# oscarknagg/wurm

Hardware: AMD Instinct MI355X
Metric: env_steps_per_s (higher is better)
Workload: dtype i32

## Files before the change

wurm_amd/csrc/options.hip:

```cpp
#include <atomic>
#include <cerrno>
#include <cstdlib>
#include <cstring>

#include "options.hpp"
#include "../../include/wurm_hip.h"

namespace wurm {

constexpr Options DEFAULTS = {1ll << 20, 12288, 6144, -1, -1, -1, 12, 0, 2048, 0, -1, 0, 0, 1, -1, -1, 0, 1024, 256};
Options opt = DEFAULTS;
std::atomic<long long> launch_count{0};

namespace {

struct Entry {
    const char *name;
    long long Options::*field;
};

const Entry table[] = {
    {"WURM_GRID_STEP_MIN_CELLS", &Options::grid_step_min_cells},
    {"WURM_LANE_STEP_MIN_ENVS", &Options::lane_step_min_envs},
    {"WURM_LANE_ROLLOUT_MIN_ENVS", &Options::lane_rollout_min_envs},
    {"WURM_LANE_ROLLOUT_EPW", &Options::lane_rollout_epw},
    {"WURM_RESIDENT_MIN_ENVS", &Options::resident_min_envs},
    {"WURM_RESIDENT_EPW", &Options::resident_epw},
    {"WURM_GRID_WAVES_PER_CU", &Options::grid_waves_per_cu},
    {"WURM_POLICY_GENERIC", &Options::policy_generic},
    {"WURM_MULTI_GROUP_MIN_ENVS", &Options::multi_group_min_envs},
    {"WURM_MULTI_GROUP_VARIANT", &Options::multi_group_variant},
    {"WURM_MULTI_GROUP_STEP_WPB", &Options::multi_group_step_wpb},
    {"WURM_MULTI_GROUP_SHAPE", &Options::multi_group_shape},
    {"WURM_GRID_ROTATE", &Options::grid_rotate},
    {"WURM_MULTI_SHAPE_KERNELS", &Options::multi_shape_kernels},
    {"WURM_GRIDWORLD_LANE_EPW", &Options::gridworld_lane_epw},
    {"WURM_GRID_ROLLOUT_MIN_SIZE", &Options::grid_rollout_min_size},
    {"WURM_POLICY_WIDE", &Options::policy_wide},
    {"WURM_S9_PAIR_MAX_ENVS", &Options::s9_pair_max_envs},
    {"WURM_S9_CROP_HELPER_MIN_STEPS", &Options::s9_crop_helper_min_steps},
};

const Entry *find(const char *name)
{
    if (!name) return nullptr;
    for (const Entry &e : table)
        if (strcmp(e.name, name) == 0) return &e;
    return nullptr;
}

bool parse_whole(const char *v, long long &out)
{
    if (!v || !*v) return false;
    errno = 0;
    char *end = nullptr;
    const long long x = strtoll(v, &end, 10);
    if (errno != 0 || end == v) return false;
    while (*end == ' ' || *end == '\t' || *end == '\n') ++end;
    if (*end != '\0') return false;
    out = x;
    return true;
}

__attribute__((constructor)) void read_environment()
{
    for (const Entry &e : table) {
        long long x;
        if (parse_whole(getenv(e.name), x)) opt.*(e.field) = x;
    }
}

}
}

extern "C" {

int wurm_set_option(const char *name, int64_t value)
{
    const wurm::Entry *e = wurm::find(name);
    if (!e) return WURM_ERR_INVALID_ARG;
    wurm::opt.*(e->field) = (long long)value;
    return WURM_OK;
}

int64_t wurm_get_option(const char *name)
{
    const wurm::Entry *e = wurm::find(name);
    return e ? (int64_t)(wurm::opt.*(e->field)) : INT64_MIN;
}

int64_t wurm_launch_count(void) { return (int64_t)wurm::launch_count.load(std::memory_order_relaxed); }

int wurm_reset_option(const char *name)
{
    const wurm::Entry *e = wurm::find(name);
    if (!e) return WURM_ERR_INVALID_ARG;
    wurm::opt.*(e->field) = wurm::DEFAULTS.*(e->field);
    return WURM_OK;
}

}
```

wurm_amd/csrc/options.hpp:

```cpp
#pragma once
#include <atomic>

namespace wurm {

struct Options {
    long long grid_step_min_cells;
    long long lane_step_min_envs;
    long long lane_rollout_min_envs;
    long long lane_rollout_epw;
    long long resident_min_envs;
    long long resident_epw;
    long long grid_waves_per_cu;
    long long policy_generic;
    long long multi_group_min_envs;
    long long multi_group_variant;
    long long multi_group_step_wpb;
    long long multi_group_shape;
    long long grid_rotate;
    long long multi_shape_kernels;
    long long gridworld_lane_epw;
    long long grid_rollout_min_size;
    long long policy_wide;
    long long s9_pair_max_envs;
    long long s9_crop_helper_min_steps;
};

extern Options opt;

extern std::atomic<long long> launch_count;
#define WURM_LAUNCH(...) do { ::wurm::launch_count.fetch_add(1, std::memory_order_relaxed); hipLaunchKernelGGL(__VA_ARGS__); } while (0)

}
```

wurm_amd/csrc/single_kernels.hpp:

```cpp
#pragma once

#include "single_device.hpp"

namespace wurm {

template <int CPL, bool SNAKE>
__global__ __launch_bounds__(256) void step_kernel(StepArgs p)
{
    const int wave = (int)(threadIdx.x >> 6), wpb = (int)(blockDim.x >> 6);
    const long long env = xcd_block(blockIdx.x, gridDim.x) * wpb + wave;
    if (env >= p.N) return;
    if (p.only_flagged && uniform((int)p.done[env]) != (int)GRID_SKIPPED) return;
    signed char *lds = wurm_lds + wave * p.lds_per_wave;
    const int NCH = SNAKE ? 3 : 2;
    const Geo g = make_geo<CPL>(p.S);
    float *envp = p.envs + env * NCH * g.C;
    Env<CPL> e;
    load_state<CPL, SNAKE>(envp, g, e);
    const long long a_in = uniform64(load_action(p.actions, p.act_dtype, env));
    const bool inj = p.inject_food != nullptr;
    const int inj_cell = inj ? uniform(p.inject_food[env]) : -1;
    StepOut out;
    step_core<CPL, SNAKE, true>(e, g, envp, a_in, out, p.seed, p.call, (u64)(p.env_offset + env), inj, inj_cell, lds);
    if (g.lane == 0) {
        if (SNAKE) {
            store_action(p.actions, p.act_dtype, env, out.action);
            p.selfc[env] = (uint8_t)out.selfc;
        }
        p.reward[env] = out.reward;
        p.done[env] = (uint8_t)out.done;
        p.edgec[env] = (uint8_t)out.edgec;
        if (p.done_copy) p.done_copy[env] = (uint8_t)out.done;
    }
    if (p.obs_mode != WURM_OBS_NONE)
        write_obs<CPL, SNAKE>(e, g, out.headcell, p.obs + env * p.obs_elems, p.obs_mode, p.obs_n, lds);
}

template <int CPL, bool SNAKE>
__global__ __launch_bounds__(256) void fused_step_kernel(StepArgs p)
{
    const int wave = (int)(threadIdx.x >> 6), wpb = (int)(blockDim.x >> 6);
    const long long env = xcd_block(blockIdx.x, gridDim.x) * wpb + wave;
    if (env >= p.N) return;
    if (p.only_flagged && uniform((int)p.done[env]) != (int)GRID_SKIPPED) return;
    fused_step_env<CPL, SNAKE>(p, env, wurm_lds + wave * p.lds_per_wave);
}

template <int CPL, bool SNAKE>
__global__ __launch_bounds__(256) void reset_kernel(StepArgs p)
{
    const int wave = (int)(threadIdx.x >> 6), wpb = (int)(blockDim.x >> 6);
    const long long env = xcd_block(blockIdx.x, gridDim.x) * wpb + wave;
    if (env >= p.N) return;
    signed char *lds = wurm_lds + wave * p.lds_per_wave;
    const int NCH = SNAKE ? 3 : 2;
    const Geo g = make_geo<CPL>(p.S);
    float *envp = p.envs + env * NCH * g.C;
    Env<CPL> e;
    const bool d = uniform((int)p.done_in[env]) != 0;
    if (d) {
        const int *inj = p.inject_reset ? p.inject_reset + env * (SNAKE ? 4 : 1) : nullptr;
        reset_core<CPL, SNAKE>(e, g, p.seed, p.call, (u64)(p.env_offset + env), inj, p.start_y, p.start_x);
        store_state<CPL, SNAKE>(envp, g, e);
    } else {
        if (p.obs_mode == WURM_OBS_NONE) return;
        load_state<CPL, SNAKE>(envp, g, e);
    }
    if (p.obs_mode != WURM_OBS_NONE)
        write_obs<CPL, SNAKE>(e, g, find_head<CPL>(e), p.obs + env * p.obs_elems, p.obs_mode, p.obs_n, lds);
}

template <int CPL, bool SNAKE>
__global__ __launch_bounds__(256) void observe_kernel(StepArgs p)
{
    const int wave = (int)(threadIdx.x >> 6), wpb = (int)(blockDim.x >> 6);
    const long long env = xcd_block(blockIdx.x, gridDim.x) * wpb + wave;
    if (env >= p.N) return;
    signed char *lds = wurm_lds + wave * p.lds_per_wave;
    const int NCH = SNAKE ? 3 : 2;
    const Geo g = make_geo<CPL>(p.S);
    Env<CPL> e;
    load_state<CPL, SNAKE>(p.envs + env * NCH * g.C, g, e);
    write_obs<CPL, SNAKE>(e, g, find_head<CPL>(e), p.obs + env * p.obs_elems, p.obs_mode, p.obs_n, lds);
}

template <int CPL, bool SNAKE, int OBSK = -1, bool INJ = true>
__global__ __launch_bounds__(256) void rollout_kernel(StepArgs p)
{
    const int wave = uniform((int)(threadIdx.x >> 6)), wpb = (int)(blockDim.x >> 6);
    const long long env = xcd_block(blockIdx.x, gridDim.x) * wpb + wave;
    if (env >= p.N) return;
    if (p.only_flagged && uniform((int)p.done[env]) != (int)GRID_SKIPPED) return;
    signed char *lds = wurm_lds + wave * p.lds_per_wave;
    const Geo g = make_geo<CPL>(p.S);
    float *envp = p.envs + env * (SNAKE ? 3 : 2) * g.C;
    Env<CPL> e;
    load_state<CPL, SNAKE>(envp, g, e);
    rollout_generic<CPL, SNAKE, OBSK, INJ>(p, env, envp, g, e, lds);
}

template <int CPL, bool SNAKE, bool ROLL>
__global__ __launch_bounds__(256) void flagged_kernel(StepArgs p)
{
    const int wave = uniform((int)(threadIdx.x >> 6)), wpb = (int)(blockDim.x >> 6), lane = (int)(threadIdx.x & 63u);
    const long long base = ((long long)blockIdx.x * wpb + wave) * 64;
    if (base >= p.N) return;
    const bool flag = base + lane < p.N && p.done[base + lane] == GRID_SKIPPED;
    signed char *lds = wurm_lds + wave * p.lds_per_wave;
    for (u64 m = ballot(flag); m != 0; m &= m - 1) {
        const long long env = base + first_bit(m);
        if constexpr (ROLL) {
            const Geo g = make_geo<CPL>(p.S);
            float *envp = p.envs + env * (SNAKE ? 3 : 2) * g.C;
            Env<CPL> e;
            load_state<CPL, SNAKE>(envp, g, e);
            rollout_generic<CPL, SNAKE, -1, true>(p, env, envp, g, e, lds);
        } else {
            fused_step_env<CPL, SNAKE>(p, env, lds);
        }
        wave_lds_sync();
    }
}


template <int OBSK, bool COMPACT>
__global__ __launch_bounds__(256) void rollout_lean_kernel(StepArgs p)
{
    constexpr int CPL = 2;
    static_assert(OBSK == WURM_OBS_PARTIAL || OBSK == WURM_OBS_NONE, "lean rollout: partial_n or no observation");
    const int wave = uniform((int)(threadIdx.x >> 6)), wpb = (int)(blockDim.x >> 6);
    const long long env = xcd_block(blockIdx.x, gridDim.x) * wpb + wave;
    if (env >= p.N) return;
    const Geo g = make_geo<CPL>(p.S);
    const int S = g.S, Sm2 = S - 2, lane = g.lane;
    float *envp = p.envs + env * 3 * g.C;
    Env<CPL> e;
    load_state<CPL, true>(envp, g, e);

    Fast f = {-1, 0, 0, 0, 0, -1};
    bool lean = fast_init<CPL>(e, g, f);
    if (lean) {
        const bool head_in = f.hc >= 0 && (unsigned)(f.hy - 1) < (unsigned)Sm2 && (unsigned)(f.hx - 1) < (unsigned)Sm2;
        int under_food = 0;
        if (f.food >= 0) under_food = lane_value(f.food >= 64 ? e.body[1] : e.body[0], f.food & 63);
        lean = head_in && under_food == 0;
    }
    if (!uniform((int)lean)) {
        rollout_generic<CPL, true, OBSK, false>(p, env, envp, g, e, wurm_lds + wave * p.lds_per_wave);
        return;
    }

    const u64 env_id = (u64)(p.env_offset + env);
    const u64 int0 = ballot((g.interior & 1) != 0), int1 = ballot((g.interior & 2) != 0);
    const float rcpSm2 = 1.0f / (float)Sm2;
    int hy1 = uniform(f.hy) - 1, hx1 = uniform(f.hx) - 1, hc = uniform(f.hc), L = uniform(f.L), o16 = uniform(f.o) << 4;
    int food = uniform(f.food);
    int foodc = food - (COMPACT ? S + 1 : 0);
    int G = L;
    int ex0 = e.body[0], ex1 = e.body[1];
    const u64 ring0 = lane_mask((g.valid & 1) != 0) & ~int0, ring1 = lane_mask((g.valid & 2) != 0) & ~int1;
    u64 X0 = ring0 | ((unsigned)food < 64u ? 1ull << food : 0), X1 = ring1 | (food >= 64 ? 1ull << (food - 64) : 0);

    const int n = OBSK == WURM_OBS_PARTIAL ? p.obs_n : 0, W = 2 * n + 1, W2 = W * W;
    const int w = min(lane, W2 - 1), wy = div_size(w, 1.0f / (float)W), wx = w - wy * W;
    const int dy0 = wy - n, dx0 = wx - n;
    const bool centre = w == n * W + n;
    const int cell_d = dy0 * S + dx0 - (COMPACT ? S + 1 : 0);
    const float green = centre ? 1.0f : 127.0f / 255.0f;
    const u32 off_r = (u32)w * 4u, off_g = (u32)(W2 + w) * 4u, off_b = (u32)(2 * W2 + w) * 4u;
    const long long obs_stride = p.N * p.obs_elems;
    float *obs_t = p.obs + env * p.obs_elems;

    for (long long t0 = 0; t0 < p.T; t0 += 64) {
        const int nt = (int)min((long long)64, p.T - t0);
        const long long my_t = t0 + lane;
        long long my_a = lane < nt ? load_action(p.actions, p.act_dtype, my_t * p.N + env) : 0;
        asm volatile("" : "+v"(my_a));
        int my_mov01, my_mov23;
        {
            const bool in_range = my_a >= 0 && my_a < 4;
            const int a_small = in_range ? (int)my_a : 7, a_mod = (int)(my_a % 4);
            int ent[4];
#pragma unroll
            for (int o = 0; o < 4; ++o) {
                const int a_out = o == a_small ? (o ^ 2) : a_mod;
                const int ai = a_out & 3, dy = -tap_y(ai), dx = -tap_x(ai);
                ent[o] = (a_out & 7) | ((ai ^ 2) << 4) | ((dy & 3) << 6) | ((dx & 3) << 8) | (((dy * S + dx) & 63) << 10);
            }
            my_mov01 = ent[0] | (ent[1] << 16);
            my_mov23 = ent[2] | (ent[3] << 16);
        }
        const u64 my_call = p.call + 2ull * (u64)my_t;
        const LeanReset my_reset = lean_reset_draw(p.seed, my_call + 1ull, env_id, S, rcpSm2);
        const int my_food = (int)rng_words(p.seed, my_call, env_id, RNG_FOOD, 0).w[0];
        int my_rec = 0, my_ate = 0, my_fl = 0;
        {
            const int T = G - L;
            ex0 = max(ex0 - T, 0);
            ex1 = max(ex1 - T, 0);
            G = L;
        }

        for (int j = 0; j < nt; ++j) {
            const u64 mov = (u64)(u32)lane_value(my_mov01, j) | ((u64)(u32)lane_value(my_mov23, j) << 32);
            const int ent = (int)(u32)(mov >> o16);
            o16 = ent & 48;
            hy1 += (ent << 24) >> 30;
            hx1 += (ent << 22) >> 30;
            hc += (ent << 16) >> 26;
            G += 1;
            asm("s_cmp_eq_u32 %1, %2\n\ts_addc_u32 %0, %0, 0" : "+s"(L) : "s"(hc), "s"(food) : "scc");
            const int T = G - L;
            const u64 p0 = lane_mask(ex0 > T), p1 = lane_mask(ex1 > T);
            ex0 = lane == hc ? G : ex0;
            ex1 = lane + 64 == hc ? G : ex1;
            const u64 special = hc >= 64 ? (p1 | X1) : (p0 | X0);
            bool finished = false, selfc = false, edgec = false;
            if (__builtin_expect(((special >> (hc & 63)) & 1) != 0, 0)) {
                if (hc == food) {
                    my_ate = lane == j ? 1 : my_ate;
                    const u64 head0 = (unsigned)hc < 64u ? 1ull << hc : 0, head1 = hc >= 64 ? 1ull << (hc - 64) : 0;
                    food = lean_food_cell(p0 | head0, p1 | head1, int0, int1, (u32)lane_value(my_food, j), lane);
                    foodc = food - (COMPACT ? S + 1 : 0);
                    X0 = ring0 | ((unsigned)food < 64u ? 1ull << food : 0);
                    X1 = ring1 | (food >= 64 ? 1ull << (food - 64) : 0);
                }
                selfc = (((hc >= 64 ? p1 : p0) >> (hc & 63)) & 1) != 0;
                edgec = max((unsigned)hy1, (unsigned)hx1) >= (unsigned)Sm2;
                finished = selfc | edgec;
            }

            if (OBSK == WURM_OBS_PARTIAL) {
                const unsigned off_grid = max((unsigned)(hy1 + dy0), (unsigned)(hx1 + dx0));
                const int cell = (COMPACT && centre) ? 63 : hc + cell_d;
                unsigned occ;
                if (COMPACT) {
                    const u64 M = (p0 >> (S + 1)) | (p1 << (63 - S)) | (1ull << 63);
                    u64 sh;
                    asm("v_lshrrev_b64 %0, %1, %2" : "=v"(sh) : "v"(cell), "s"(M));
                    occ = (u32)sh & 1u;
                } else {
                    occ = ((u32)((cell < 64 ? p0 : p1) >> (cell & 63)) & 1u) | (centre ? 1u : 0u);
                }
                const float vr = (off_grid | (occ << 30)) < (unsigned)Sm2 ? 1.0f : 0.0f;
                const float vb = cell == foodc ? 0.0f : vr;
                const float vg = (off_grid | ((occ ^ 1u) << 30)) < (unsigned)Sm2 ? green : vb;
                asm volatile("global_store_dword %0, %1, %2" : : "v"(off_r), "v"(vr), "s"(obs_t) : "memory");
                asm volatile("global_store_dword %0, %1, %2" : : "v"(off_g), "v"(vg), "s"(obs_t) : "memory");
                asm volatile("global_store_dword %0, %1, %2" : : "v"(off_b), "v"(vb), "s"(obs_t) : "memory");
                obs_t += obs_stride;
            }
            my_rec = set_lane(my_rec, ent, j);

            if (__builtin_expect(finished, 0)) {
                my_fl = lane == j ? (selfc ? 1 : 0) | (edgec ? 2 : 0) : my_fl;
                const int ra = lane_value(my_reset.a, j), rb = lane_value(my_reset.b, j);
                hy1 = (ra & 15) - 1; hx1 = ((ra >> 4) & 15) - 1; o16 = ((ra >> 8) & 3) << 4; food = ra >> 10;
                foodc = food - (COMPACT ? S + 1 : 0);
                X0 = ring0 | ((unsigned)food < 64u ? 1ull << food : 0);
                X1 = ring1 | (food >= 64 ? 1ull << (food - 64) : 0);
                hc = rb & 127;
                const int sc = (rb >> 7) & 127, tc = rb >> 14;
                const int c1 = lane + 64;
                ex0 = lane == tc ? T + 1 : 0; ex0 = lane == sc ? T + 2 : ex0; ex0 = lane == hc ? T + 3 : ex0;
                ex1 = c1 == tc ? T + 1 : 0;   ex1 = c1 == sc ? T + 2 : ex1;   ex1 = c1 == hc ? T + 3 : ex1;
                L = 3;
                G = T + 3;
            }
        }
        if (lane < nt) {
            const long long i = my_t * p.N + env;
            store_action(p.actions, p.act_dtype, i, (long long)((my_rec << 29) >> 29));
            p.reward[i] = my_ate ? 1.0f : 0.0f;
            p.done[i] = (uint8_t)(my_fl != 0);
            p.selfc[i] = (uint8_t)(my_fl & 1);
            p.edgec[i] = (uint8_t)(my_fl >> 1);
        }
    }
    const int T = G - L;
    e.body[0] = max(ex0 - T, 0);
    e.body[1] = max(ex1 - T, 0);
    f.hc = hc; f.hy = hy1 + 1; f.hx = hx1 + 1; f.L = L; f.o = o16 >> 4; f.food = food;
    fast_sync_bits<CPL>(e, g, f);
    store_state<CPL, true>(envp, g, e);
}


template <int OBSK, bool INJ = false, bool PAIR = false, bool CROPH = false>
__global__ __launch_bounds__(256) void rollout_s9_kernel(StepArgs p)
{
    constexpr int CPL = 2, S = 9;
    static_assert(OBSK == WURM_OBS_PARTIAL || OBSK == WURM_OBS_NONE, "9x9 rollout: partial_n or no observation");
    static_assert(!CROPH || (PAIR && OBSK == WURM_OBS_PARTIAL), "9x9 rollout: the helper renders the crops of the pair form");
    const int wave = uniform((int)(threadIdx.x >> 6)), wpb = (int)(blockDim.x >> 6);
    const long long env = PAIR ? xcd_block(blockIdx.x, gridDim.x) : xcd_block(blockIdx.x, gridDim.x) * wpb + wave;
    if (env >= p.N) return;
    const Geo g = make_geo<CPL>(S);
    const int lane = g.lane;
    const u64 env_id = (u64)(p.env_offset + env);
    WURM_TL_DECL;
    WURM_TL(0);
    WURM_TL(6);

    const auto chunk_draw = [&](const long long t0, const int nt) __attribute__((always_inline)) {
        S9Chunk ch;
        const long long my_t = t0 + lane;
        long long my_a = lane < nt ? load_action(p.actions, p.act_dtype, my_t * p.N + env) : 0;
        asm volatile("" : "+v"(my_a));
        if constexpr (!PAIR) WURM_TL_LAP(1);
        {
            const auto entry = [](int a_out) {
                const int ai = a_out & 3;
                return ((ai ^ 2) << 4) | (((-tap_y(ai) * 8 - tap_x(ai)) & 63) << 6) | ((a_out & 7) << 12);
            };
            const bool in_range = my_a >= 0 && my_a < 4;
            const int a_small = in_range ? (int)my_a : 7, a_mod = (int)(my_a % 4);
            int me[4];
#pragma unroll
            for (int o = 0; o < 4; ++o)
                me[o] = entry(o == a_small ? (o ^ 2) : a_mod);
            ch.mov01 = me[0] | (me[1] << 16);
            ch.mov23 = me[2] | (me[3] << 16);
        }
        const u64 my_call = p.call + 2ull * (u64)my_t;
        if constexpr (INJ) {
            int sy = 4, sx = 4, d = 0, fc = -1, fe = -1;
            if (lane < nt) {
                const int *ir = p.inject_reset + (my_t * p.N + env) * 4;
                sy = ir[0]; sx = ir[1]; d = ir[2]; fc = ir[3];
                fe = p.inject_food[my_t * p.N + env];
            }
            asm volatile("" : "+v"(sy), "+v"(sx), "+v"(d), "+v"(fc), "+v"(fe));
            d &= 3;
            const int sc = sy * 8 + sx, dc = tap_y(d) * 8 + tap_x(d);
            const int fcy = div_size(max(fc, 0), g.rcpS), fey = div_size(max(fe, 0), g.rcpS);
            const int fcode = (fc >= 0 && fc < S * S) ? fcy * 8 + (fc - fcy * S) : -1;
            ch.reset.a = d | (fcode << 2);
            ch.reset.b = (sc + dc) | (sc << 7) | ((sc - dc) << 14);
            ch.food = (fe >= 0 && fe < S * S) ? fey * 8 + (fe - fey * S) : -1;
        } else {
            ch.reset = s9_reset_draw(p.seed, my_call + 1ull, env_id);
            ch.food = (int)rng_words(p.seed, my_call, env_id, RNG_FOOD, 0).w[0];
        }
        return ch;
    };
    const auto flush = [&](const long long t0, const int nt, const int act, const int ate, const int fl) __attribute__((always_inline)) {
        if (lane < nt) {
            const long long i = (t0 + lane) * p.N + env;
            store_action(p.actions, p.act_dtype, i, (long long)act);
            p.reward[i] = ate ? 1.0f : 0.0f;
            p.done[i] = (uint8_t)(fl != 0);
            p.selfc[i] = (uint8_t)(fl & 1);
            p.edgec[i] = (uint8_t)(fl >> 1);
        }
    };

    int *const pair_lds = (int *)(wurm_lds + p.lds_per_wave);
    constexpr int PAIR_CHUNK = 5 * 64, PAIR_REC = 2 * PAIR_CHUNK, PAIR_RECSZ = CROPH ? 4 * 64 : 64, PAIR_LEAN = PAIR_REC + 2 * PAIR_RECSZ;
    const long long n_chunks = (p.T + 63) >> 6;
    if constexpr (PAIR) {
        if (wave != 0) {
            const auto draw_into = [&](const long long k) __attribute__((always_inline)) {
                const long long t0 = k << 6;
                const S9Chunk ch = chunk_draw(t0, (int)min((long long)64, p.T - t0));
                int *cb = pair_lds + (int)(k & 1) * PAIR_CHUNK + lane;
                cb[0] = ch.mov01; cb[64] = ch.mov23; cb[128] = ch.reset.a; cb[192] = ch.reset.b; cb[256] = ch.food;
            };
            const auto flush_from = [&](const long long k) __attribute__((always_inline)) {
                const long long t0 = k << 6;
                const int rec = pair_lds[PAIR_REC + (int)(k & 1) * PAIR_RECSZ + lane];
                flush(t0, (int)min((long long)64, p.T - t0), (rec << 29) >> 29, (rec >> 3) & 1, rec >> 4);
            };
            int spp = 1, sub = 0;
            S9Window win = {};
            if constexpr (CROPH) {
#ifndef WURM_S9_CROP_SPP1
                spp = (2 * p.obs_n + 1) * (2 * p.obs_n + 1) <= 32 ? 2 : 1;
#endif
                sub = spp == 2 ? lane >> 5 : 0;
                win = s9_window(spp == 2 ? lane & 31 : lane, p.obs_n);
            }
            const auto render = [&](const long long k) __attribute__((always_inline)) {
                const int W2 = (2 * p.obs_n + 1) * (2 * p.obs_n + 1);
                const long long t0 = k << 6, obs_stride = p.N * p.obs_elems;
                const int nt = (int)min((long long)64, p.T - t0);
                const int *rb = pair_lds + PAIR_REC + (int)(k & 1) * PAIR_RECSZ;
                const int centre = win.code_d == 0 ? 1 : 0, code_d1 = win.code_d + 1;
                float *obs_t = p.obs + (t0 * p.N + env) * p.obs_elems;
                const auto pass = [&](const int j, const int my_sub) __attribute__((always_inline)) {
                    const int sj = j + my_sub;
                    const int w1 = rb[64 + sj];
                    const u64 body = (u64)(u32)rb[128 + sj] | ((u64)(u32)rb[192 + sj] << 32);
                    const int c = w1 & 127;
                    unsigned inside = (u32)(win.live_tab >> (w1 & 63)) & 1u;
                    const bool edge = ((w1 >> 26) & 1) != 0;
                    if (lane_mask(edge) != 0) {
                        const int ai = (w1 >> 22) & 3, pc = c - ((w1 << 10) >> 26);
                        const int hy = (pc >> 3) - tap_y(ai), hx = (pc & 7) - tap_x(ai);
                        const unsigned e_inside = max((unsigned)(hy + win.dy0 - 1), (unsigned)(hx + win.dx0 - 1)) < 7u ? 1u : 0u;
                        inside = edge ? e_inside : inside;
                    }
                    const unsigned taken = ((u32)(body >> ((w1 + win.code_d) & 63)) & 1u) | (u32)centre;
                    const unsigned both = inside & taken;
                    const int code1 = c + code_d1, food1 = (w1 >> 7) & 127;
                    const float vr = inside > taken ? 1.0f : 0.0f;
                    const float vb = code1 != food1 ? vr : 0.0f;
                    const float vg = both != 0 ? win.green : vb;
                    const u32 o = (u32)((long long)my_sub * obs_stride * 4) + (u32)win.w * 4u;
                    float *const obs_s = (float *)uniform64((long long)obs_t);
                    asm volatile("global_store_dword %0, %1, %6\n\tglobal_store_dword %2, %3, %6\n\tglobal_store_dword %4, %5, %6"
                                 : : "v"(o), "v"(vr), "v"(o + (u32)W2 * 4u), "v"(vg), "v"(o + (u32)W2 * 8u), "v"(vb), "s"(obs_s) : "memory");
                };
                int j = 0;
                for (; j + spp <= nt; j += spp) {
                    pass(j, sub);
                    obs_t += spp * obs_stride;
                }
                if (j < nt) pass(j, 0);
            };
            if (n_chunks > 0) draw_into(0);
            pair_barrier();
            if (uniform(pair_lds[PAIR_LEAN]) == 0) return;
            for (long long k = 0; k < n_chunks; ++k) {
                if (k + 1 < n_chunks) draw_into(k + 1);
                if (k > 0) flush_from(k - 1);
                if constexpr (CROPH) {
                    WURM_TL_LAP(1);
                    if (k > 0) render(k - 1);
                    WURM_TL_LAP(2);
                }
                pair_barrier();
                if constexpr (CROPH) WURM_TL_LAP(3);
            }
            if (n_chunks > 0) flush_from(n_chunks - 1);
            if constexpr (CROPH) {
                WURM_TL_LAP(1);
                if (n_chunks > 0) render(n_chunks - 1);
                WURM_TL_LAP(4);
                if (p.T > 1) WURM_TL_STORE(p.obs + (p.N + env) * p.obs_elems, lane);
            }
            return;
        }
    }

    float *envp = p.envs + env * 3 * (S * S);
    Env<CPL> e;
    load_state<CPL, true>(envp, g, e);

    Fast f = {-1, 0, 0, 0, 0, -1};
    bool lean = fast_init<CPL>(e, g, f);
    if (lean) {
        const bool head_in = f.hc >= 0 && (unsigned)(f.hy - 1) < 7u && (unsigned)(f.hx - 1) < 7u;
        const int fy = f.food >= 0 ? div_size(f.food, g.rcpS) : 1, fx = f.food >= 0 ? f.food - fy * S : 1;
        const bool food_in = (unsigned)(fy - 1) < 7u && (unsigned)(fx - 1) < 7u;
        int under_food = 0;
        if (f.food >= 0) under_food = lane_value(f.food >= 64 ? e.body[1] : e.body[0], f.food & 63);
        const bool ring_body = lane_mask((e.body[0] > 0 && !(g.interior & 1)) || (e.body[1] > 0 && !(g.interior & 2))) != 0;
        lean = head_in && food_in && under_food == 0 && !ring_body;
    }
    if constexpr (PAIR) {
        if (lane == 0) pair_lds[PAIR_LEAN] = lean ? 1 : 0;
        pair_barrier();
    }
    if (!uniform((int)lean)) {
        rollout_generic<CPL, true, OBSK, INJ, true>(p, env, envp, g, e, wurm_lds + wave * p.lds_per_wave);
        return;
    }

    const int ly = lane >> 3, lx = lane & 7;
    const bool lane_in = ly >= 1 && lx >= 1;
    const int my_cell = ly * S + lx;
    const u64 RING = ~lane_mask(lane_in);
    int ex = lane_in ? __float2int_rn(envp[2 * S * S + my_cell]) : 0;
    int c = uniform(f.hy) * 8 + uniform(f.hx), ent = uniform(f.o) << 4;
    int foodc = -1;
    if (f.food >= 0) {
        const int fy = uniform(div_size(f.food, g.rcpS));
        foodc = fy * 8 + (uniform(f.food) - fy * S);
    }
    u64 XF = RING | (foodc >= 0 ? 1ull << foodc : 0);
    int G = uniform(f.L), T1 = 1;

    const int n = OBSK == WURM_OBS_PARTIAL ? p.obs_n : 0, W = 2 * n + 1, W2 = W * W;
    const int w = min(lane, W2 - 1), wy = div_size(w, 1.0f / (float)W), wx = w - wy * W;
    const int dy0 = wy - n, dx0 = wx - n;
    const int code_d = dy0 * 8 + dx0;
    const float green = (w == n * W + n) ? 1.0f : 127.0f / 255.0f;
    u64 live_tab = 0;
#pragma unroll
    for (int y = 1; y <= 7; ++y) {
        u32 cols = 0;
#pragma unroll
        for (int x = 1; x <= 7; ++x)
            if ((unsigned)(x + dx0 - 1) < 7u) cols |= 1u << x;
        if ((unsigned)(y + dy0 - 1) < 7u) live_tab |= (u64)cols << (8 * y);
    }
    const u32 off_r = (u32)w * 4u, off_g = (u32)(W2 + w) * 4u, off_b = (u32)(2 * W2 + w) * 4u;
    const long long obs_stride = p.N * p.obs_elems;
    float *obs_t = p.obs + env * p.obs_elems;

    WURM_TL_LAP(5);
    for (long long t0 = 0; t0 < p.T; t0 += 64) {
        const int nt = (int)min((long long)64, p.T - t0);
        int my_mov01, my_mov23, my_food;
        S9Reset my_reset;
        if constexpr (PAIR) {
            const int *cb = pair_lds + (int)((t0 >> 6) & 1) * PAIR_CHUNK + lane;
            my_mov01 = cb[0]; my_mov23 = cb[64]; my_reset.a = cb[128]; my_reset.b = cb[192]; my_food = cb[256];
            asm volatile("" : "+v"(my_mov01), "+v"(my_mov23), "+v"(my_reset.a), "+v"(my_reset.b), "+v"(my_food));
            WURM_TL_LAP(1);
        } else {
            const S9Chunk ch = chunk_draw(t0, nt);
            my_mov01 = ch.mov01; my_mov23 = ch.mov23; my_reset = ch.reset; my_food = ch.food;
#ifdef WURM_TIMELINE
            asm volatile("" : "+v"(my_mov01), "+v"(my_mov23), "+v"(my_reset.a), "+v"(my_reset.b), "+v"(my_food));
#endif
            WURM_TL_LAP(2);
        }
        int my_rec = 0, my_ate = 0, my_fl = 0;
        S9CropRec crop_rec = {0, 0, 0, 0, 0};
        {
            const int T = T1 - 1;
            ex = max(ex - T, 0);
            G -= T;
            T1 = 1;
        }

        const auto step = [&](const int j) __attribute__((always_inline)) {
            const u64 body_moved = lane_mask(ex > T1);
            const u64 mov = (u64)(u32)lane_value(my_mov01, j) | ((u64)(u32)lane_value(my_mov23, j) << 32);
            ent = (int)(u32)(mov >> (ent & 63));
            if constexpr (!CROPH) my_rec = set_lane(my_rec, ent, j);
            asm("s_add_i32 %0, %0, %1" : "+s"(c) : "s"((ent << 20) >> 26) : "scc");
            G += 1;
            asm("s_cmp_lg_u32 %1, %2\n\ts_addc_u32 %0, %0, 0" : "+s"(T1) : "s"(c), "s"(foodc) : "scc");
            if constexpr (CROPH) set_lane(crop_rec, ent, c, foodc, body_moved, j);
            u64 body = body_moved;
            const u64 head = 1ull << (c & 63);
            ex = keep_in_lane(ex, G, head);
            u64 occ = body | head;

            unsigned inside = 0;
            int code = c + code_d;
            u64 mask = occ;
            if (OBSK == WURM_OBS_PARTIAL && !CROPH) {
                u64 lv;
                asm("v_lshrrev_b64 %0, %1, %2" : "=v"(lv) : "s"(c), "v"(live_tab));
                inside = (u32)lv & 1u;
            }

            int shown_food = foodc;
            if (__builtin_expect((((body | XF) >> (c & 63)) & 1) != 0, 0)) {
                const u64 lane_j = 1ull << (j & 63);
                if (c == foodc) {
                    my_ate = keep_in_lane(my_ate, 1, lane_j);
                    occ = lane_mask(ex > T1 - 1);
                    body = occ & ~head;
                    mask = occ;
                    if constexpr (INJ) {
                        foodc = lane_value(my_food, j);
                    } else {
                        const u64 fr = ~(occ | RING);
                        const int n_free = popc64(fr);
                        foodc = -1;
                        if (n_free > 0) {
                            const int K = (int)mulhi_range((u32)lane_value(my_food, j), (u32)n_free);
                            foodc = first_bit(lane_mask((int)((fr >> lane) & 1) & (int)(rank_below(fr) == K)));
                        }
                    }
                    XF = RING | (foodc >= 0 ? 1ull << foodc : 0);
                    if constexpr (CROPH) {
                        crop_rec.food = set_lane(crop_rec.food, foodc, j);
                        crop_rec.body_lo = set_lane(crop_rec.body_lo, (int)(u32)body, j);
                        crop_rec.body_hi = set_lane(crop_rec.body_hi, (int)(u32)(body >> 32), j);
                    }
                }
                shown_food = foodc;
                const int event = ((RING >> (c & 63)) & 1) ? 2 : ((body >> (c & 63)) & 1) ? 1 : 0;
                if (OBSK == WURM_OBS_PARTIAL && !CROPH && event == 2) {
                    const int ai = (ent >> 12) & 3, pc = c - ((ent << 20) >> 26);
                    const int hy = (pc >> 3) - tap_y(ai), hx = (pc & 7) - tap_x(ai);
                    inside = max((unsigned)(hy + dy0 - 1), (unsigned)(hx + dx0 - 1)) < 7u ? 1u : 0u;
                    code = (hy + dy0) * 8 + hx + dx0;
                    mask = body;
                }
                if (event != 0) {
                    my_fl = keep_in_lane(my_fl, event, lane_j);
                    const int ra = lane_value(my_reset.a, j), rb = lane_value(my_reset.b, j);
                    ent = (ra & 3) << 4;
                    foodc = ra >> 2;
                    XF = INJ ? (RING | (foodc >= 0 ? 1ull << foodc : 0)) : (RING | (1ull << foodc));
                    c = rb & 127;
                    const int sc = (rb >> 7) & 127, tc = rb >> 14;
                    ex = lane == tc ? T1 : 0; ex = lane == sc ? T1 + 1 : ex; ex = lane == c ? T1 + 2 : ex;
                    G = T1 + 2;
                }
            }

            if (OBSK == WURM_OBS_PARTIAL && !CROPH) {
                u64 sh;
                asm("v_lshrrev_b64 %0, %1, %2" : "=v"(sh) : "v"(code), "s"(mask));
                const unsigned taken = (u32)sh & 1u;
                const unsigned both = inside & taken;
                float vr, vb, vg;
                u64 m_free, m_not_food, m_taken;
                asm("v_cmp_gt_u32_e64 %3, %6, %7\n\t"
                    "v_cmp_ne_u32_e64 %4, %8, %9\n\t"
                    "v_cmp_ne_u32_e64 %5, 0, %10\n\t"
                    "v_cndmask_b32_e64 %0, 0, 1.0, %3\n\t"
                    "v_cndmask_b32_e64 %1, 0, %0, %4\n\t"
                    "v_cndmask_b32_e64 %2, %1, %11, %5"
                    : "=&v"(vr), "=&v"(vb), "=&v"(vg), "=&s"(m_free), "=&s"(m_not_food), "=&s"(m_taken)
                    : "v"(inside), "v"(taken), "s"(shown_food), "v"(code), "v"(both), "v"(green));
                asm volatile("global_store_dword %0, %1, %6\n\tglobal_store_dword %2, %3, %6\n\tglobal_store_dword %4, %5, %6"
                             : : "v"(off_r), "v"(vr), "v"(off_g), "v"(vg), "v"(off_b), "v"(vb), "s"(obs_t) : "memory");
                obs_t += obs_stride;
            }
        };
        constexpr int U = 4;
        const int nu = nt & -U;
        int j = 0;
        for (; j != nu; j += U) {
#pragma unroll
            for (int u = 0; u < U; ++u) step(j + u);
        }
        for (; j < nt; ++j) step(j);
        WURM_TL_LAP(3);
        if constexpr (PAIR) {
            if constexpr (CROPH) {
                int *rb = pair_lds + PAIR_REC + (int)((t0 >> 6) & 1) * PAIR_RECSZ + lane;
                my_rec = crop_rec.ent;
                rb[64] = (crop_rec.c & 127) | (((crop_rec.food + 1) & 127) << 7) | (((my_rec >> 4) & 0x7FF) << 14) | ((my_fl & 3) << 25);
                rb[128] = crop_rec.body_lo;
                rb[192] = crop_rec.body_hi;
                rb[0] = ((my_rec >> 12) & 7) | (my_ate << 3) | (my_fl << 4);
            } else {
                pair_lds[PAIR_REC + (int)((t0 >> 6) & 1) * 64 + lane] = ((my_rec >> 12) & 7) | (my_ate << 3) | (my_fl << 4);
            }
            pair_barrier();
        } else {
            flush(t0, nt, (my_rec << 17) >> 29, my_ate, my_fl);
        }
        WURM_TL_LAP(4);
    }
    if (OBSK == WURM_OBS_PARTIAL && (!CROPH || p.T > 64)) WURM_TL_STORE(p.obs + env * p.obs_elems, lane);
    if (lane_in) {
        envp[my_cell] = lane == foodc ? 1.0f : 0.0f;
        envp[S * S + my_cell] = lane == c ? 1.0f : 0.0f;
        envp[2 * S * S + my_cell] = (float)max(ex - (T1 - 1), 0);
    }
}

template <int CPL>
__global__ __launch_bounds__(256) void check_kernel(const float *__restrict__ envs, uint32_t *__restrict__ err,
                                                    long long N, int S)
{
    const int wave = (int)(threadIdx.x >> 6), wpb = (int)(blockDim.x >> 6);
    const long long env = xcd_block(blockIdx.x, gridDim.x) * wpb + wave;
    if (env >= N) return;
    const Geo g = make_geo<CPL>(S);
    const float *envp = envs + env * 3 * g.C;
    int bad_food = 0;
    float hs = 0.0f, bs = 0.0f, bm = -INFINITY, hb = 0.0f, hf = 0.0f, fs = 0.0f;
#pragma unroll
    for (int k = 0; k < CPL; ++k) {
        int c = g.lane + 64 * k;
        if ((g.valid >> k) & 1) {
            float f = envp[c], h = envp[g.C + c], b = envp[2 * g.C + c];
            bad_food |= !(f == 0.0f || f == 1.0f);
            hs += h; bs += b; hb += h * b; hf += h * f; fs += f;
            bm = fmaxf(bm, b);
        }
    }
    bad_food = ballot(bad_food != 0) != 0;
#pragma unroll
    for (int sh = 32; sh >= 1; sh >>= 1) {
        hs += __shfl_xor(hs, sh); bs += __shfl_xor(bs, sh); hb += __shfl_xor(hb, sh); hf += __shfl_xor(hf, sh);
        fs += __shfl_xor(fs, sh); bm = fmaxf(bm, __shfl_xor(bm, sh));
    }
    uint32_t m = 0;
    if (bad_food) m |= WURM_CHK_FOOD_VALUE;
    if (hs != 1.0f) m |= WURM_CHK_ONE_HEAD;
    if (!(bs > 0.0f)) m |= WURM_CHK_HAS_SNAKE;
    if (bm != hb) m |= WURM_CHK_HEAD_AT_END;
    if ((__fsqrt_rn(8.0f * bs + 1.0f) - 1.0f) / 2.0f != bm) m |= WURM_CHK_BODY_RANGE;
    if (!(bs >= 6.0f)) m |= WURM_CHK_MIN_LENGTH;
    if (hf != 0.0f) m |= WURM_CHK_HEAD_ON_FOOD;
    if (fs != 1.0f) m |= WURM_CHK_ONE_FOOD;
    if (g.lane == 0) err[env] = m;
}

template <int CPL>
__global__ __launch_bounds__(256) void orientations_kernel(const float *__restrict__ envs, long long *__restrict__ out,
                                                           long long N, int S, int lds_per_wave)
{
    const int wave = (int)(threadIdx.x >> 6), wpb = (int)(blockDim.x >> 6);
    const long long env = xcd_block(blockIdx.x, gridDim.x) * wpb + wave;
    if (env >= N) return;
    signed char *lds = wurm_lds + wave * lds_per_wave;
    const Geo g = make_geo<CPL>(S);
    Env<CPL> e;
    load_state<CPL, true>(envs + env * 3 * g.C, g, e);
    int lm = 0;
#pragma unroll
    for (int k = 0; k < CPL; ++k) lm = max(lm, e.body[k]);
    const int L = uniform(wave_max_i32(lm));
    const int o = orientation_of<CPL>(e, g, L, lds);
    if (g.lane == 0) out[env] = o;
}

}
```

wurm_amd/csrc/single_launch.hpp:

```cpp
#pragma once

#include "single_kernels.hpp"
#include "lane_step.hpp"

namespace wurm {

enum Kind { K_STEP, K_RESET, K_OBSERVE, K_ROLLOUT, K_FUSED };

enum Route { R_GENERIC, R_GRID_STEP, R_LANE_STEP, R_GRID_ROLLOUT, R_LANE_ROLLOUT, R_LANE_WIDE, R_S9_INJ, R_S9, R_LEAN, R_GENERIC_PARTIAL, R_GENERIC_NONE, R_LANE_RESIDENT, R_LANE_WIDE_RESIDENT, R_GRIDWORLD_LANE, R_GRIDWORLD_LANE_STEP };
extern thread_local Route last_route;
extern thread_local int last_waves_per_env;
extern thread_local int last_crop_wave;

static const char *route_name(Route r)
{
    switch (r) {
    case R_GRID_STEP: return "grid_step";
    case R_LANE_STEP: return "lane_step";
    case R_GRID_ROLLOUT: return "grid_rollout";
    case R_LANE_ROLLOUT: return "lane_rollout";
    case R_LANE_WIDE: return "lane_wide";
    case R_S9_INJ: return "rollout_s9_injected";
    case R_S9: return "rollout_s9";
    case R_LEAN: return "rollout_lean";
    case R_GENERIC_PARTIAL: return "rollout_generic_partial";
    case R_GENERIC_NONE: return "rollout_generic_none";
    case R_LANE_RESIDENT: return "lane_resident";
    case R_LANE_WIDE_RESIDENT: return "lane_wide_resident";
    case R_GRIDWORLD_LANE: return "gridworld_lane";
    case R_GRIDWORLD_LANE_STEP: return "gridworld_lane_step";
    default: return "generic";
    }
}

static Route route_of(Kind kind, bool snake, int cpl, const StepArgs &p)
{
    const bool stepish = kind == K_STEP || kind == K_FUSED;
    if (snake && cpl >= 4 && stepish && grid_step_eligible(p) &&
        (p.N * (long long)p.S * p.S >= opt.grid_step_min_cells || p.resident != nullptr)) return R_GRID_STEP;
    if (snake && cpl == 2 && stepish && p.N >= opt.lane_step_min_envs && lane_step_eligible(p)) return R_LANE_STEP;
    if (kind == K_ROLLOUT && !snake && gridworld_lane_eligible(p)) return R_GRIDWORLD_LANE;
    if (stepish && !snake && gridworld_lane_step_eligible(p)) return R_GRIDWORLD_LANE_STEP;
    if (kind != K_ROLLOUT || !snake) return R_GENERIC;
    if (cpl >= 4) return grid_rollout_eligible(p) ? R_GRID_ROLLOUT : R_GENERIC;
    if (p.N >= opt.lane_rollout_min_envs && lane_rollout_eligible(p)) return R_LANE_ROLLOUT;
    if (p.N >= opt.lane_rollout_min_envs && lane_wide_eligible(p)) return R_LANE_WIDE;
    const bool rng_mode = p.inject_food == nullptr && p.inject_reset == nullptr;
    const bool injected = p.inject_food != nullptr && p.inject_reset != nullptr;
    const bool small_crop_or_none = (p.obs_mode == WURM_OBS_PARTIAL && p.obs_n <= 3) || p.obs_mode == WURM_OBS_NONE;
    if (injected && p.S == 9 && small_crop_or_none) return R_S9_INJ;
    if (rng_mode && p.S == 9 && small_crop_or_none) return R_S9;
    if (rng_mode && p.S > 9 && small_crop_or_none) return R_LEAN;
    if (rng_mode && p.obs_mode == WURM_OBS_PARTIAL && p.obs_n <= 6) return R_GENERIC_PARTIAL;
    if (rng_mode && p.obs_mode == WURM_OBS_NONE) return R_GENERIC_NONE;
    return R_GENERIC;
}

template <int CPL, bool SNAKE>
static hipError_t launch_one(Kind kind, const StepArgs &p, dim3 grid, dim3 block, size_t lds, hipStream_t st)
{
    (void)hipGetLastError();
    const Route route = route_of(kind, SNAKE, CPL, p);
    last_route = route;
    last_waves_per_env = 1;
    last_crop_wave = 0;
    const unsigned wpb_f = block.x / 64u;
    const dim3 fgrid((unsigned)((p.N + 64ll * wpb_f - 1) / (64ll * wpb_f)));
    switch (route) {
    case R_GRID_STEP:
        if constexpr (SNAKE && CPL >= 4) {
            hipError_t err = launch_grid_step(p, st);
            if (err != hipSuccess) return err;
            WURM_LAUNCH((flagged_kernel<CPL, SNAKE, false>), fgrid, block, lds, st, p);
        }
        break;
    case R_LANE_STEP:
        if constexpr (SNAKE && CPL == 2) return launch_lane_step(p, st);
        break;
    case R_GRID_ROLLOUT:
        if constexpr (SNAKE && CPL >= 4) {
            hipError_t err = launch_grid_rollout(p, st);
            if (err != hipSuccess) return err;
            WURM_LAUNCH((flagged_kernel<CPL, SNAKE, true>), fgrid, block, lds, st, p);
        }
        break;
    case R_LANE_ROLLOUT:
        if constexpr (SNAKE && CPL == 2) return launch_lane_rollout(p, st);
        break;
    case R_LANE_WIDE:
        if constexpr (SNAKE && CPL == 2) return launch_lane_wide(p, st);
        break;
    case R_GRIDWORLD_LANE:
        if constexpr (!SNAKE) {
            hipError_t err = launch_gridworld_lane_rollout(p, st);
            if (err != hipSuccess) return err;
            if (!(p.resident != nullptr && p.resident_valid))
                WURM_LAUNCH((flagged_kernel<CPL, SNAKE, true>), fgrid, block, lds, st, p);
        }
        break;
    case R_GRIDWORLD_LANE_STEP:
        if constexpr (!SNAKE) {
            hipError_t err = launch_gridworld_lane_step(p, st);
            if (err != hipSuccess) return err;
            if (!(p.resident != nullptr && p.resident_valid))
                WURM_LAUNCH((flagged_kernel<CPL, SNAKE, false>), fgrid, block, lds, st, p);
        }
        break;
    case R_S9_INJ:
    case R_S9:
        if constexpr (SNAKE && CPL == 2) {
            const bool inj = route == R_S9_INJ, none = p.obs_mode == WURM_OBS_NONE;
            if (p.N <= opt.s9_pair_max_envs) {
                const dim3 pgrid((unsigned)p.N), pblock(128);
                const size_t plds = (size_t)p.lds_per_wave + (2 * 5 * 64 + 2 * 64 + 4) * sizeof(int);
                last_waves_per_env = 2;
                if (!none && opt.s9_crop_helper_min_steps >= 0 && p.T >= opt.s9_crop_helper_min_steps &&
                    p.N * p.obs_elems * 4 < (1ll << 31)) {
                    const size_t clds = (size_t)p.lds_per_wave + (2 * 5 * 64 + 2 * 4 * 64 + 4) * sizeof(int);
                    last_crop_wave = 1;
                    if (inj) WURM_LAUNCH((rollout_s9_kernel<WURM_OBS_PARTIAL, true, true, true>), pgrid, pblock, clds, st, p);
                    else WURM_LAUNCH((rollout_s9_kernel<WURM_OBS_PARTIAL, false, true, true>), pgrid, pblock, clds, st, p);
                } else
                if (inj && none) WURM_LAUNCH((rollout_s9_kernel<WURM_OBS_NONE, true, true>), pgrid, pblock, plds, st, p);
                else if (inj) WURM_LAUNCH((rollout_s9_kernel<WURM_OBS_PARTIAL, true, true>), pgrid, pblock, plds, st, p);
                else if (none) WURM_LAUNCH((rollout_s9_kernel<WURM_OBS_NONE, false, true>), pgrid, pblock, plds, st, p);
                else WURM_LAUNCH((rollout_s9_kernel<WURM_OBS_PARTIAL, false, true>), pgrid, pblock, plds, st, p);
            } else if (inj) {
                if (none) WURM_LAUNCH((rollout_s9_kernel<WURM_OBS_NONE, true>), grid, block, lds, st, p);
                else WURM_LAUNCH((rollout_s9_kernel<WURM_OBS_PARTIAL, true>), grid, block, lds, st, p);
            } else {
                if (none) WURM_LAUNCH((rollout_s9_kernel<WURM_OBS_NONE>), grid, block, lds, st, p);
                else WURM_LAUNCH((rollout_s9_kernel<WURM_OBS_PARTIAL>), grid, block, lds, st, p);
            }
        }
        break;
    case R_LEAN:
        if constexpr (SNAKE && CPL == 2) {
            if (p.obs_mode == WURM_OBS_NONE) WURM_LAUNCH((rollout_lean_kernel<WURM_OBS_NONE, false>), grid, block, lds, st, p);
            else WURM_LAUNCH((rollout_lean_kernel<WURM_OBS_PARTIAL, false>), grid, block, lds, st, p);
        }
        break;
    case R_GENERIC_PARTIAL:
        if constexpr (SNAKE && CPL == 2) WURM_LAUNCH((rollout_kernel<CPL, SNAKE, WURM_OBS_PARTIAL, false>), grid, block, lds, st, p);
        break;
    case R_GENERIC_NONE:
        if constexpr (SNAKE && CPL == 2) WURM_LAUNCH((rollout_kernel<CPL, SNAKE, WURM_OBS_NONE, false>), grid, block, lds, st, p);
        break;
    case R_LANE_RESIDENT:
    case R_LANE_WIDE_RESIDENT:
    case R_GENERIC:
        switch (kind) {
        case K_STEP: WURM_LAUNCH((step_kernel<CPL, SNAKE>), grid, block, lds, st, p); break;
        case K_RESET: WURM_LAUNCH((reset_kernel<CPL, SNAKE>), grid, block, lds, st, p); break;
        case K_OBSERVE: WURM_LAUNCH((observe_kernel<CPL, SNAKE>), grid, block, lds, st, p); break;
        case K_FUSED: WURM_LAUNCH((fused_step_kernel<CPL, SNAKE>), grid, block, lds, st, p); break;
        case K_ROLLOUT: WURM_LAUNCH((rollout_kernel<CPL, SNAKE>), grid, block, lds, st, p); break;
        }
        break;
    }
    return hipGetLastError();
}

template <bool SNAKE>
int launch(Kind kind, StepArgs p, void *stream)
{
    if (p.N == 0) return WURM_OK;
    const int cpl = pick_cpl(p.S);
    if (cpl < 0) return WURM_ERR_UNSUPPORTED;
    const int wpb = p.N <= 4096 ? 1 : 4;
    p.lds_per_wave = ((p.S * p.S + 15) / 16) * 16;
    dim3 block(64 * wpb), grid((unsigned)((p.N + wpb - 1) / wpb));
    size_t lds = (size_t)p.lds_per_wave * wpb;
    hipStream_t st = (hipStream_t)stream;
    hipError_t err;
    switch (cpl) {
    case 2: err = launch_one<2, SNAKE>(kind, p, grid, block, lds, st); break;
    case 4: err = launch_one<4, SNAKE>(kind, p, grid, block, lds, st); break;
    case 8: err = launch_one<8, SNAKE>(kind, p, grid, block, lds, st); break;
    case 16: err = launch_one<16, SNAKE>(kind, p, grid, block, lds, st); break;
    case 24: err = launch_one<24, SNAKE>(kind, p, grid, block, lds, st); break;
    case 32: err = launch_one<32, SNAKE>(kind, p, grid, block, lds, st); break;
    case 48: err = launch_one<48, SNAKE>(kind, p, grid, block, lds, st); break;
    default: err = launch_one<64, SNAKE>(kind, p, grid, block, lds, st); break;
    }
    return err == hipSuccess ? WURM_OK : WURM_ERR_HIP;
}

}
```

Baseline: 4.418 billion.

## Add third render-only wave to 9x9 pair rollout for small env counts

After: 4.874 billion (median of 6 runs). 1.1x the previous value.

```diff
diff --git a/wurm_amd/csrc/options.hip b/wurm_amd/csrc/options.hip
--- a/wurm_amd/csrc/options.hip
+++ b/wurm_amd/csrc/options.hip
@@ -8,7 +8,7 @@
 
 namespace wurm {
 
-constexpr Options DEFAULTS = {1ll << 20, 12288, 6144, -1, -1, -1, 12, 0, 2048, 0, -1, 0, 0, 1, -1, -1, 0, 1024, 256};
+constexpr Options DEFAULTS = {1ll << 20, 12288, 6144, -1, -1, -1, 12, 0, 2048, 0, -1, 0, 0, 1, -1, -1, 0, 1024, 256, 512, 512};
 Options opt = DEFAULTS;
 std::atomic<long long> launch_count{0};
 
@@ -39,6 +39,8 @@
     {"WURM_POLICY_WIDE", &Options::policy_wide},
     {"WURM_S9_PAIR_MAX_ENVS", &Options::s9_pair_max_envs},
     {"WURM_S9_CROP_HELPER_MIN_STEPS", &Options::s9_crop_helper_min_steps},
+    {"WURM_S9_TRIO_MAX_ENVS", &Options::s9_trio_max_envs},
+    {"WURM_S9_TRIO_MIN_STEPS", &Options::s9_trio_min_steps},
 };
 
 const Entry *find(const char *name)
diff --git a/wurm_amd/csrc/options.hpp b/wurm_amd/csrc/options.hpp
--- a/wurm_amd/csrc/options.hpp
+++ b/wurm_amd/csrc/options.hpp
@@ -23,6 +23,8 @@
     long long policy_wide;
     long long s9_pair_max_envs;
     long long s9_crop_helper_min_steps;
+    long long s9_trio_max_envs;
+    long long s9_trio_min_steps;
 };
 
 extern Options opt;
diff --git a/wurm_amd/csrc/single_kernels.hpp b/wurm_amd/csrc/single_kernels.hpp
--- a/wurm_amd/csrc/single_kernels.hpp
+++ b/wurm_amd/csrc/single_kernels.hpp
@@ -286,12 +286,14 @@
 }
 
 
-template <int OBSK, bool INJ = false, bool PAIR = false, bool CROPH = false>
+template <int OBSK, bool INJ = false, bool PAIR = false, bool CROPH = false, int RW = 1>
 __global__ __launch_bounds__(256) void rollout_s9_kernel(StepArgs p)
 {
     constexpr int CPL = 2, S = 9;
+    constexpr int S9_TRIO_SHARE = 24, S9_TRIO_LAST_SHARE = 32;
     static_assert(OBSK == WURM_OBS_PARTIAL || OBSK == WURM_OBS_NONE, "9x9 rollout: partial_n or no observation");
     static_assert(!CROPH || (PAIR && OBSK == WURM_OBS_PARTIAL), "9x9 rollout: the helper renders the crops of the pair form");
+    static_assert(RW == 1 || (RW == 2 && CROPH), "9x9 rollout: a second render wave beside a helper that renders");
     const int wave = uniform((int)(threadIdx.x >> 6)), wpb = (int)(blockDim.x >> 6);
     const long long env = PAIR ? xcd_block(blockIdx.x, gridDim.x) : xcd_block(blockIdx.x, gridDim.x) * wpb + wave;
     if (env >= p.N) return;
@@ -360,6 +362,7 @@
     const long long n_chunks = (p.T + 63) >> 6;
     if constexpr (PAIR) {
         if (wave != 0) {
+            const bool renders_only = RW == 2 && wave == 2;
             const auto draw_into = [&](const long long k) __attribute__((always_inline)) {
                 const long long t0 = k << 6;
                 const S9Chunk ch = chunk_draw(t0, (int)min((long long)64, p.T - t0));
@@ -380,13 +383,15 @@
                 sub = spp == 2 ? lane >> 5 : 0;
                 win = s9_window(spp == 2 ? lane & 31 : lane, p.obs_n);
             }
-            const auto render = [&](const long long k) __attribute__((always_inline)) {
+            const auto render = [&](const long long k, const int share) __attribute__((always_inline)) {
                 const int W2 = (2 * p.obs_n + 1) * (2 * p.obs_n + 1);
                 const long long t0 = k << 6, obs_stride = p.N * p.obs_elems;
                 const int nt = (int)min((long long)64, p.T - t0);
+                const int split = RW == 2 ? ((nt * share) >> 6) & ~1 : nt;
+                const int j0 = renders_only ? split : 0, j1 = renders_only ? nt : split;
                 const int *rb = pair_lds + PAIR_REC + (int)(k & 1) * PAIR_RECSZ;
                 const int centre = win.code_d == 0 ? 1 : 0, code_d1 = win.code_d + 1;
-                float *obs_t = p.obs + (t0 * p.N + env) * p.obs_elems;
+                float *obs_t = p.obs + ((t0 + j0) * p.N + env) * p.obs_elems;
                 const auto pass = [&](const int j, const int my_sub) __attribute__((always_inline)) {
                     const int sj = j + my_sub;
                     const int w1 = rb[64 + sj];
@@ -411,33 +416,35 @@
                     asm volatile("global_store_dword %0, %1, %6\n\tglobal_store_dword %2, %3, %6\n\tglobal_store_dword %4, %5, %6"
                                  : : "v"(o), "v"(vr), "v"(o + (u32)W2 * 4u), "v"(vg), "v"(o + (u32)W2 * 8u), "v"(vb), "s"(obs_s) : "memory");
                 };
-                int j = 0;
-                for (; j + spp <= nt; j += spp) {
+                int j = j0;
+                for (; j + spp <= j1; j += spp) {
                     pass(j, sub);
                     obs_t += spp * obs_stride;
                 }
-                if (j < nt) pass(j, 0);
+                if (j < j1) pass(j, 0);
             };
-            if (n_chunks > 0) draw_into(0);
+            if (n_chunks > 0 && !renders_only) draw_into(0);
             pair_barrier();
             if (uniform(pair_lds[PAIR_LEAN]) == 0) return;
             for (long long k = 0; k < n_chunks; ++k) {
-                if (k + 1 < n_chunks) draw_into(k + 1);
-                if (k > 0) flush_from(k - 1);
+                if (!renders_only) {
+                    if (k + 1 < n_chunks) draw_into(k + 1);
+                    if (k > 0) flush_from(k - 1);
+                }
                 if constexpr (CROPH) {
                     WURM_TL_LAP(1);
-                    if (k > 0) render(k - 1);
+                    if (k > 0) render(k - 1, S9_TRIO_SHARE);
                     WURM_TL_LAP(2);
                 }
                 pair_barrier();
                 if constexpr (CROPH) WURM_TL_LAP(3);
             }
-            if (n_chunks > 0) flush_from(n_chunks - 1);
+            if (n_chunks > 0 && !renders_only) flush_from(n_chunks - 1);
             if constexpr (CROPH) {
                 WURM_TL_LAP(1);
-                if (n_chunks > 0) render(n_chunks - 1);
+                if (n_chunks > 0) render(n_chunks - 1, S9_TRIO_LAST_SHARE);
                 WURM_TL_LAP(4);
-                if (p.T > 1) WURM_TL_STORE(p.obs + (p.N + env) * p.obs_elems, lane);
+                if (p.T > wave) WURM_TL_STORE(p.obs + (wave * p.N + env) * p.obs_elems, lane);
             }
             return;
         }
diff --git a/wurm_amd/csrc/single_launch.hpp b/wurm_amd/csrc/single_launch.hpp
--- a/wurm_amd/csrc/single_launch.hpp
+++ b/wurm_amd/csrc/single_launch.hpp
@@ -118,6 +118,12 @@
                     p.N * p.obs_elems * 4 < (1ll << 31)) {
                     const size_t clds = (size_t)p.lds_per_wave + (2 * 5 * 64 + 2 * 4 * 64 + 4) * sizeof(int);
                     last_crop_wave = 1;
+                    if (p.N <= opt.s9_trio_max_envs && opt.s9_trio_min_steps >= 0 && p.T >= opt.s9_trio_min_steps) {
+                        const dim3 tblock(192);
+                        last_waves_per_env = 3;
+                        if (inj) WURM_LAUNCH((rollout_s9_kernel<WURM_OBS_PARTIAL, true, true, true, 2>), pgrid, tblock, clds, st, p);
+                        else WURM_LAUNCH((rollout_s9_kernel<WURM_OBS_PARTIAL, false, true, true, 2>), pgrid, tblock, clds, st, p);
+                    } else
                     if (inj) WURM_LAUNCH((rollout_s9_kernel<WURM_OBS_PARTIAL, true, true, true>), pgrid, pblock, clds, st, p);
                     else WURM_LAUNCH((rollout_s9_kernel<WURM_OBS_PARTIAL, false, true, true>), pgrid, pblock, clds, st, p);
                 } else
```
